# jonassibbesen/rpvg

Hardware: AMD Instinct MI355X
Metric: read-pairs quantified/sec (higher is better)
Workload: dtype f64

## Files before the change

### rpvg_amd/csrc/em_plan.hpp

```cpp
#ifndef RPVG_EM_PLAN_HPP
#define RPVG_EM_PLAN_HPP

#include <algorithm>
#include <cstddef>
#include <cstdint>

#ifndef RPVG_PLAN_FN
#if defined(__HIPCC__)
#define RPVG_PLAN_FN __host__ __device__ inline
#else
#define RPVG_PLAN_FN inline
#endif
#endif

namespace rpvg_em {

constexpr int kEmBins = 12;
constexpr int kEmGridBin = 11;
constexpr int kEmWideBin = 10;
constexpr int kEmWorkBuckets = 32;
constexpr uint32_t kEmMidGridMax = 8;
constexpr uint32_t kEmMidGridLog2 = 16;
constexpr uint32_t kEmMidBuckets = kEmWorkBuckets - kEmMidGridLog2;
constexpr int kEmStreamedBin = 3;
// ... 5 lines not shown

RPVG_PLAN_FN size_t emLdsBytes(uint32_t cols, uint32_t rows, uint32_t entries, int block, bool resident) {
    size_t bytes = sizeof(double) * ((1 + static_cast<size_t>(block) / 64) * cols + block / 64 + 2);
    if (resident) bytes += static_cast<size_t>(rows) * 16 + static_cast<size_t>(entries) * 8 + (static_cast<size_t>(rows) + 1 + entries) * 4 + 8;
    return (bytes + 15) & ~static_cast<size_t>(15);
}

RPVG_PLAN_FN size_t emGridLdsBytes(const uint32_t cols) { return sizeof(double) * 5 * static_cast<size_t>(cols); }

RPVG_PLAN_FN size_t emRegisterLdsBytes(const int rpl, const int cols) { return (64 * static_cast<size_t>(rpl) * cols + 2) * sizeof(double); }

struct EmBinRule {
    uint32_t use_register_kernel;
    uint64_t streamed_small_work;
    uint64_t grid_min_work;
};

RPVG_PLAN_FN int emBinOf(const EmBinRule rule, const uint32_t C, const uint32_t rows, const uint32_t entries) {
    const uint64_t work = static_cast<uint64_t>(entries) + rows;
    if (rule.grid_min_work != 0 && work >= rule.grid_min_work && emGridLdsBytes(C) <= kEmLdsLimit) return kEmGridBin;
    if (rule.use_register_kernel && C <= 16 && rows <= 256) return rows <= 64 ? 4 : rows <= 128 ? 5 : 6;
    if (rule.use_register_kernel && C <= kRegColsMax && rows <= 128) return rows <= 64 ? 8 : 9;
    if (emLdsBytes(C, rows, entries, 64, true) <= 8 * 1024) return 0;
    if (emLdsBytes(C, rows, entries, 256, true) <= 40 * 1024) return 1;
    if (emLdsBytes(C, rows, entries, 1024, true) <= 152 * 1024) return 7;
    if (emLdsBytes(C, 0, 0, 256, false) > kEmLdsLimit) return kEmWideBin;
    if (emLdsBytes(C, 0, 0, 1024, false) > kEmLdsLimit) return 2;
    return work <= rule.streamed_small_work ? 2 : 3;
}

RPVG_PLAN_FN uint32_t emWorkBucket(const uint32_t rows, const uint32_t entries) {
    uint64_t work = static_cast<uint64_t>(entries) + rows + 1;
    uint32_t lg = 0;
    while (work > 1 && lg < static_cast<uint32_t>(kEmWorkBuckets - 1)) {
        work >>= 1;
        ++lg;
    }
    return static_cast<uint32_t>(kEmWorkBuckets - 1) - lg;
}

RPVG_PLAN_FN bool emIsMidSize(const uint32_t bin, const uint32_t bucket) { return bin == static_cast<uint32_t>(kEmStreamedBin) && bucket < kEmMidBuckets; }
RPVG_PLAN_FN bool emMidGridAllowed(const uint64_t grid_min_work) { return grid_min_work > (1ull << kEmMidGridLog2); }
RPVG_PLAN_FN bool emMidGridMoves(const bool allowed, const uint32_t mid) { return allowed && mid > 0 && mid <= kEmMidGridMax; }
RPVG_PLAN_FN int emRouteOf(const int bin, const uint32_t bucket, const bool moved) {
    return moved && emIsMidSize(static_cast<uint32_t>(bin), bucket) ? kEmGridBin : bin;
}

RPVG_PLAN_FN bool emIsRegisterBin(const int bin) { return bin == 4 || bin == 5 || bin == 6 || bin == 8 || bin == 9; }
RPVG_PLAN_FN int emStatsSlot(const int bin, const bool one_register_launch) {
    return emIsRegisterBin(bin) && one_register_launch ? static_cast<int>(kRegisterKernelIndex) : bin;
}

constexpr int kEmMaxFusedDense = 4;
constexpr uint32_t kEmDenseMaxCols = 2048;
RPVG_PLAN_FN bool emDenseRule(const uint32_t columns, const uint32_t rows, const uint32_t entries) {
    if (columns > kEmDenseMaxCols || columns < 2) return false;
    const uint64_t ld = (static_cast<uint64_t>(columns) + 1) & ~1ull;
    return 8ull * rows * ld <= 12ull * entries + 20ull * rows;
}

constexpr uint32_t kLdsMapPaths = 16384;
constexpr uint32_t kFillSegmentRows = 1024;
constexpr uint64_t kFillLongRowEntries = 32;
constexpr size_t kFillLongRowLds = kFillSegmentRows * (3 * sizeof(uint32_t) + sizeof(double));
constexpr size_t kFillDenseLds = kFillSegmentRows * 2 * sizeof(uint32_t);
constexpr uint64_t kFillLongRowMinWork = 1ull << 18;
RPVG_PLAN_FN size_t emFillDenseLdsBytes(const uint32_t lds_map_paths, const uint64_t widest_ld) {
    return lds_map_paths * sizeof(int32_t) + kFillDenseLds + 4 * static_cast<size_t>(widest_ld) * sizeof(double);
}

struct EmSolveKnobs {
    EmBinRule rule = {1u, 0, 1ull << 18};
    bool no_collapse = false;
    bool no_fused_dense = false;
    bool register_copies = true;
    bool one_register_launch = true;
    bool fill_thread_rows = false;
    double grid_scale = 1.0;
    bool few_streams = false;
    bool launch_early = false;
    bool wait_sort_only = false;
    bool join_on_stream = false;
    bool collapse_debug = false;
    bool has_bound_bytes = false;
    uint64_t bound_bytes = 0;
};

RPVG_PLAN_FN bool emStorageByBound(const uint64_t rows_bound, const uint64_t entries_bound, const uint64_t budget) {
    return rows_bound * 20 + entries_bound * 12 <= budget;
}
template <typename Count>
inline void emStorageBases(const Count * rows, const Count * entries, const uint32_t P, uint64_t * row_base, uint64_t * ent_base, uint64_t * rows_total,
                           uint64_t * entries_total) {
    uint64_t r = 0, e = 0;
    for (uint32_t p = 0; p < P; ++p) {
        row_base[p] = r;
        ent_base[p] = e;
        r += rows[p];
        e += entries[p];
    }
    *rows_total = r;
    *entries_total = e;
}

constexpr size_t kGibbsOneWorkgroupLdsLimit = 160 * 1024;
RPVG_PLAN_FN size_t gibbsOneWorkgroupLds(const uint32_t columns) {
    return (sizeof(double) * (2 * static_cast<size_t>(columns) + 256 / 64 + 2) + 15) & ~static_cast<size_t>(15);
}
RPVG_PLAN_FN bool gibbsTakesGrid(const uint32_t columns, const uint32_t rows, const uint32_t entries, const uint64_t grid_min_work) {
    const bool too_wide = gibbsOneWorkgroupLds(columns) > kGibbsOneWorkgroupLdsLimit;
    const bool too_large = grid_min_work != 0 && static_cast<uint64_t>(rows) + entries >= grid_min_work;
    return too_wide || too_large;
}
RPVG_PLAN_FN bool gibbsGridPossible(const uint32_t max_cols, const uint64_t max_cluster_work, const uint64_t grid_min_work) {
    return gibbsOneWorkgroupLds(max_cols) > kGibbsOneWorkgroupLdsLimit || (grid_min_work != 0 && max_cluster_work >= grid_min_work);
}

struct EmSolveShape {
    uint32_t P = 0, items_bound = 0, max_cols = 0, max_cluster_paths = 0;
    uint64_t max_cluster_work = 0, rows_capacity = 0;
    unsigned long long wide_capacity = 0;
    uint32_t cus = 0;
    int side_streams = 6;
    int hardware_queues = 4;
    bool collapse_wanted = false;
};
constexpr int kEmSideStreams = 6;
constexpr uint32_t kEmCollapseMaxProblems = (1u << 20) - 2;
constexpr uint64_t kEmCollapseMaxRows = 0x7fffffffull;

struct EmFillPlan {
    uint32_t fill_grid = 0;
    uint32_t dense_grid = 0;
    uint32_t lds_map_paths = 0;
    bool long_row_scratch = false;
    size_t fill_lds = 0;
};
inline EmFillPlan planEmFill(const EmSolveShape & s, const EmSolveKnobs & knobs) {
    EmFillPlan f;
    f.fill_grid = std::min<uint32_t>(s.items_bound, s.cus * 8);
    f.dense_grid = std::min<uint32_t>(s.items_bound, s.cus * 4);
    f.lds_map_paths = (std::min<uint32_t>(s.max_cluster_paths, kLdsMapPaths) + 3) & ~3u;
    f.long_row_scratch = !knobs.fill_thread_rows && s.max_cluster_work >= kFillLongRowMinWork;
    f.fill_lds = f.lds_map_paths * sizeof(int32_t) + (f.long_row_scratch ? kFillLongRowLds : 0);
    return f;
}

enum class EmVariant : uint8_t {
    kSparse64Resident, kSparse256Resident, kSparse1024Resident, kSparse256Streamed, kSparse1024Streamed, kSparseWide,
    kRegisterBins,
    kRegister1x16, kRegister2x16, kRegister4x16, kRegister1x32, kRegister2x32
};
constexpr int kEmMainStream = -1;
struct EmLaunch {
    uint32_t bin;
    EmVariant variant;
    uint32_t grid;
    size_t lds;
    int stream;
};
inline bool operator==(const EmLaunch & a, const EmLaunch & b) {
    return a.bin == b.bin && a.variant == b.variant && a.grid == b.grid && a.lds == b.lds && a.stream == b.stream;
}
constexpr int kEmMaxLaunches = 11;

struct EmSolvePlan {
// ... 70 lines not shown
```

### rpvg_amd/csrc/em_sparse.hip

```cpp

#include "common.hpp"

#include "em_block.hpp"

#include <algorithm>
#include <memory>
#include <numeric>

using namespace rpvg_hip_detail;

namespace {

constexpr double kMinEmAbundance = 1e-8;
constexpr uint32_t kMinEmConvIts = 10;
static_assert(kEmBins == RPVG_HIP_EM_KERNELS, "a statistics slot per size bin (em_plan.hpp)");

struct EmQueues {
    uint32_t histogram[kEmBins * kEmWorkBuckets];
    uint32_t bucket_cursor[kEmBins * kEmWorkBuckets];
    uint32_t bin_start[kEmBins];
    uint32_t bin_count[kEmBins];
    uint32_t bin_cursor[kEmBins];
    uint32_t pad;
    unsigned long long wide_cursor;
    unsigned long long wide_overflow;
};


struct FillArgs {
    uint32_t num_problems;
    const uint32_t * num_problems_dev;
    uint32_t num_items;
    const uint32_t * num_items_dev;
    const uint64_t * seg_first;
    const uint32_t * item_problem;
    const uint32_t * prob_cluster;
    const uint32_t * col_path;
    const uint64_t * cluster_row_off;
    const uint64_t * cluster_path_off;
    const uint64_t * row_ent_off;
    const uint32_t * ent_path;
    const double * ent_prob;
    const double * row_count;
    const double * row_noise;
    EmProblemsView problems;
    uint32_t * seg_rows;
    uint32_t * seg_entries;
    double * seg_zero_mass;
    double * seg_total_mass;
    uint32_t * kept_entries;
    uint32_t * prob_bucket;
    EmQueues * queues;
    EmBinRule rule;
    uint32_t lds_map_paths;
    uint32_t long_row_scratch;
    uint32_t num_fused;
    EmFusedDense fused[kEmMaxFusedDense];
};

__device__ inline bool fillLongRows(const FillArgs & args, const uint32_t k) {
    const uint64_t c0 = args.cluster_row_off[k], c1 = args.cluster_row_off[k + 1];
    return args.long_row_scratch && args.row_ent_off[c1] - args.row_ent_off[c0] >= kFillLongRowEntries * (c1 - c0);
}

template <bool WRITE>
__global__ __launch_bounds__(256) void fillSegmentsKernel(const FillArgs args) {
    constexpr int BLOCK = 256;
    extern __shared__ __attribute__((aligned(16))) int32_t lds_map[];
    __shared__ uint32_t scratch[2 * (BLOCK / 64)];
    __shared__ double dscratch[BLOCK / 64];
    const uint32_t num_items = args.num_items_dev ? *args.num_items_dev : args.num_items;
    uint32_t mapped_problem = UINT32_MAX;
    for (uint32_t item = blockIdx.x; item < num_items; item += gridDim.x) {
        const uint32_t p = args.item_problem[item];
        if (WRITE) {
            bool fused = false;
            for (uint32_t f = 0; f < args.num_fused; ++f) fused = fused || args.fused[f].problem == p;
            if (fused) continue;
        }
        const uint32_t segment = static_cast<uint32_t>(item - args.seg_first[p]);
        const uint32_t k = args.prob_cluster[p];
        const uint32_t n_paths = static_cast<uint32_t>(args.cluster_path_off[k + 1] - args.cluster_path_off[k]);
        const uint32_t * cols = args.col_path + args.problems.col_off[p];
        const uint32_t n_cols = args.problems.paths(p);
        const bool use_map = n_paths <= args.lds_map_paths;
        const bool identity = n_cols == n_paths;
// ... 402 lines not shown
        if (c1 < kCells) start[c1] = excl + h0;
        if (threadIdx.x == 255) start[kCells] = before + incl;
    }
    __syncthreads();
    if (blockIdx.x == 0 && threadIdx.x < kEmBins) {
        queues->bin_start[threadIdx.x] = start[threadIdx.x * kEmWorkBuckets];
        queues->bin_count[threadIdx.x] = start[(threadIdx.x + 1) * kEmWorkBuckets] - start[threadIdx.x * kEmWorkBuckets];
    }
    const uint32_t p = blockIdx.x * blockDim.x + threadIdx.x;
    if (p >= P) return;
    uint32_t cell = prob_bucket[p];
    if (cell / kEmWorkBuckets == kEmStreamedBin && cell % kEmWorkBuckets < moved) cell = kEmGridBin * kEmWorkBuckets + cell % kEmWorkBuckets;
    order[start[cell] + atomicAdd(&queues->bucket_cursor[cell], 1u)] = p;
    if (cell / kEmWorkBuckets == 10) {
        const unsigned long long need = 2ull * (static_cast<unsigned long long>(col_off[p + 1] - col_off[p]) + 1);
        const unsigned long long at = atomicAdd(&queues->wide_cursor, need);
        wide_off[p] = at;
        if (at + need > wide_capacity) atomicAdd(&queues->wide_overflow, 1ull);
    }
}

struct GridDescribeArgs {
    const EmQueues * queues;
    const uint32_t * order;
    EmProblemsView problems;
    const uint32_t * kept_entries;
    EmGridProblem * out;
    uint32_t capacity;
};

__global__ __launch_bounds__(256) void emGridDescribeKernel(const GridDescribeArgs args) {
    const uint32_t i = blockIdx.x * blockDim.x + threadIdx.x;
    if (i >= args.queues->bin_count[kEmGridBin] || i >= args.capacity) return;
    const uint32_t p = args.order[args.queues->bin_start[kEmGridBin] + i];
    EmGridProblem d;
    d.problem = p;
    const EmProblemsView & v = args.problems;
    d.columns = v.paths(p) + 1;
    d.rows = v.kept_rows[p];
    d.entries = args.kept_entries[p];
    d.merged = (v.problem_merged != nullptr && v.problem_merged[p] != 0) ? 1u : 0u;
    d.pad = 0;
    d.row_base = v.row_base[p];
    d.ent_base = v.ent_base[p];
    d.col_begin = v.col_off[p];
    d.total_mass = v.total_mass[p];
    d.zero_mass = v.zero_mass[p];
    args.out[i] = d;
}


struct EmLaunchArgs {
    const uint32_t * order;
    EmQueues * queues;
    uint32_t bin;
    EmProblemsView problems;
    uint32_t max_em_its;
    uint32_t register_copies;
    double max_rel_em_conv;
    double * wide_vectors;
    const unsigned long long * wide_off;
    unsigned long long wide_capacity;
    double * abundances;
    double * noise_count;
    uint32_t * iterations;
};

template <int BLOCK>
__device__ __forceinline__ uint32_t nextProblem(const EmLaunchArgs & args, uint32_t * slot) {
    uint32_t i;
    if (BLOCK == 64) {
        i = (threadIdx.x == 0) ? atomicAdd(&args.queues->bin_cursor[args.bin], 1u) : 0u;
        i = static_cast<uint32_t>(__builtin_amdgcn_readfirstlane(static_cast<int>(i)));
    } else {
        __syncthreads();
        if (threadIdx.x == 0) *slot = atomicAdd(&args.queues->bin_cursor[args.bin], 1u);
        __syncthreads();
        i = *slot;
    }
    if (i >= args.queues->bin_count[args.bin]) return UINT32_MAX;
    return args.order[args.queues->bin_start[args.bin] + i];
}

template <int BLOCK, bool RESIDENT, bool WIDE>
__device__ __forceinline__ void emSparseProblem(const EmLaunchArgs & args, const uint32_t p, unsigned char * smem_raw) {
    const uint32_t C = args.problems.paths(p) + 1;
    if (WIDE && args.wide_off[p] + 2ull * C > args.wide_capacity) return;
    constexpr uint32_t kCopies = WIDE ? 1 : BLOCK / 64;
    double * a = WIDE ? args.wide_vectors + args.wide_off[p] : reinterpret_cast<double *>(smem_raw);
    double * t = a + C;
    double * red = WIDE ? reinterpret_cast<double *>(smem_raw) : t + static_cast<size_t>(kCopies) * C;
    double * tw = t + static_cast<size_t>(kCopies == 1 ? 0 : threadIdx.x >> 6) * C;

    const EmProblemRows csr = args.problems.mergedRows(p);
    const uint32_t n_rows = csr.rows;
    const uint32_t * off = csr.off;
    const double * cnt = csr.count;
    const double * nzv = csr.noise;
    const uint32_t * col = csr.col;
    const double * val = csr.val;
    if (RESIDENT) {
        const uint32_t n_ent = off[n_rows];
        double * l_cnt = red + (BLOCK / 64 + 2);
        double * l_nz = l_cnt + n_rows;
        double * l_val = l_nz + n_rows;
        uint32_t * l_off = reinterpret_cast<uint32_t *>(l_val + n_ent);
        uint32_t * l_col = l_off + (n_rows + 1);
        for (uint32_t r = threadIdx.x; r < n_rows; r += BLOCK) {
            l_cnt[r] = cnt[r];
            l_nz[r] = nzv[r];
        }
        for (uint32_t r = threadIdx.x; r <= n_rows; r += BLOCK) l_off[r] = off[r];
        for (uint32_t e = threadIdx.x; e < n_ent; e += BLOCK) {
            l_val[e] = val[e];
            l_col[e] = col[e];
        }
        off = l_off;
        cnt = l_cnt;
        nzv = l_nz;
        col = l_col;
        val = l_val;
    }
    const double T = args.problems.total_mass[p];
    const double Z = args.problems.zero_mass[p];
    const double eps = args.max_rel_em_conv;
    const uint32_t noise_col = C - 1;

    const double a0 = static_cast<double>(1.0f / static_cast<float>(C));
    for (uint32_t j = threadIdx.x; j < C; j += BLOCK) a[j] = a0;

    for (uint32_t j = threadIdx.x; j < kCopies * C; j += BLOCK) t[j] = 0;
    __syncthreads();

    const double inv_T = 1.0 / T;
    uint32_t iters = 0, conv = 0;
    for (uint32_t it = 0; it < args.max_em_its; ++it) {
        const double a_noise = a[noise_col];
        double tn = 0;
        for (uint32_t r = threadIdx.x; r < n_rows; r += BLOCK) {
            const uint32_t e0 = off[r], e1 = off[r + 1];
            const double nz = nzv[r];
            double s = nz * a_noise;
            for (uint32_t e = e0; e < e1; ++e) s += val[e] * a[col[e]];
            double y = __builtin_amdgcn_rcp(s);
            y = fma(fma(-s, y, 1.0), y, y);
            y = fma(fma(-s, y, 1.0), y, y);
            const double quot = cnt[r] * y;
            const double w = cnt[r] == 0.0 ? 0.0 : fma(fma(-s, quot, cnt[r]), y, quot);
            for (uint32_t e = e0; e < e1; ++e) atomicAdd(&tw[col[e]], w * val[e]);
            tn += w * nz;
        }
        tn = waveSumF64(tn);
        if ((threadIdx.x & 63) == 0 && tn != 0.0) atomicAdd(&tw[noise_col], tn);
        __syncthreads();
        int viol = 0;
        for (uint32_t j = threadIdx.x; j < C; j += BLOCK) {
            const double aj = a[j];
            double tj = t[j];
            t[j] = 0;
#pragma unroll
            for (uint32_t w = 1; w < kCopies; ++w) {
                tj += t[w * C + j];
                t[w * C + j] = 0;
            }
            const double an = (j == noise_col) ? (aj * tj + Z) * inv_T : (aj * tj) * inv_T;
            if (an >= kMinEmAbundance && fabs(an - aj) > eps * an) viol = 1;
            a[j] = an;
        }
        int any_viol;
        if (BLOCK == 64) {
            any_viol = __any(viol);
            __syncthreads();
        } else {
            any_viol = __syncthreads_or(viol);
        }
        ++iters;
        if (!any_viol) {
            if (++conv == kMinEmConvIts) break;
        } else {
            conv = 0;
        }
    }

    double low = 0;
    double * out = args.abundances + args.problems.col_off[p];
    for (uint32_t j = threadIdx.x; j < noise_col; j += BLOCK) {
        const double aj = a[j];
        if (aj < kMinEmAbundance) {
            low += aj * T;
            out[j] = 0;
        } else {
            out[j] = aj * T;
        }
    }
    low = blockReduceSum<double, BLOCK>(low, red);
    if (threadIdx.x == 0) {
        args.noise_count[p] = low + a[noise_col] * T;
        args.iterations[p] = iters;
    }
}

template <int BLOCK, bool RESIDENT, bool WIDE = false>
__global__ __launch_bounds__(BLOCK) void emSparseKernel(const EmLaunchArgs args) {
    extern __shared__ __attribute__((aligned(16))) unsigned char smem_raw[];
    __shared__ uint32_t next_slot;
    if (blockIdx.x >= args.queues->bin_count[args.bin]) return;
    for (uint32_t p = nextProblem<BLOCK>(args, &next_slot); p != UINT32_MAX; p = nextProblem<BLOCK>(args, &next_slot)) {
        emSparseProblem<BLOCK, RESIDENT, WIDE>(args, p, smem_raw);
        if (BLOCK == 64) __syncthreads();
    }
}

template <int BLOCK, bool RESIDENT, bool WIDE = false>
hipError_t launchEm(const EmLaunchArgs & args, uint32_t grid, size_t lds, hipStream_t stream) {
    if (grid == 0) return hipSuccess;
    if (lds > kLdsOptIn) {
        hipError_t e = hipFuncSetAttribute(reinterpret_cast<const void *>(&emSparseKernel<BLOCK, RESIDENT, WIDE>),
                                           hipFuncAttributeMaxDynamicSharedMemorySize, static_cast<int>(lds));
        if (e != hipSuccess) return e;
    }
    emSparseKernel<BLOCK, RESIDENT, WIDE><<<dim3(grid), dim3(BLOCK), lds, stream>>>(args);
    return hipGetLastError();
}


template <int D>
__device__ __forceinline__ double quadSwapF64(const double v) {
    constexpr int perm = (D == 1) ? 0xB1 : 0x4E;
    const int lo = __builtin_amdgcn_mov_dpp(__double2loint(v), perm, 0xF, 0xF, true);
    const int hi = __builtin_amdgcn_mov_dpp(__double2hiint(v), perm, 0xF, 0xF, true);
    return __hiloint2double(hi, lo);
}

__device__ __forceinline__ void swapHalvesF64(double & x, double & y) {
    const auto lo = __builtin_amdgcn_permlane32_swap(static_cast<unsigned>(__double2loint(x)), static_cast<unsigned>(__double2loint(y)), false, false);
    const auto hi = __builtin_amdgcn_permlane32_swap(static_cast<unsigned>(__double2hiint(x)), static_cast<unsigned>(__double2hiint(y)), false, false);
    x = __hiloint2double(static_cast<int>(hi[0]), static_cast<int>(lo[0]));
    y = __hiloint2double(static_cast<int>(hi[1]), static_cast<int>(lo[1]));
}

__device__ __forceinline__ void swapRowsF64(double & x, double & y) {
    const auto lo = __builtin_amdgcn_permlane16_swap(static_cast<unsigned>(__double2loint(x)), static_cast<unsigned>(__double2loint(y)), false, false);
    const auto hi = __builtin_amdgcn_permlane16_swap(static_cast<unsigned>(__double2hiint(x)), static_cast<unsigned>(__double2hiint(y)), false, false);
    x = __hiloint2double(static_cast<int>(hi[0]), static_cast<int>(lo[0]));
    y = __hiloint2double(static_cast<int>(hi[1]), static_cast<int>(lo[1]));
}

template <int CTRL>
__device__ __forceinline__ double halveF64(const double x, const double y, const bool upper) {
    const double send = upper ? x : y, keep = upper ? y : x;
    const int lo = __builtin_amdgcn_mov_dpp(__double2loint(send), CTRL, 0xF, 0xF, true);
    const int hi = __builtin_amdgcn_mov_dpp(__double2hiint(send), CTRL, 0xF, 0xF, true);
    return keep + __hiloint2double(hi, lo);
}

template <int COLS, int SKIP = 0>
__device__ __forceinline__ double columnSumsOverWave(double (&v)[COLS], const uint32_t lane) {
    if (SKIP < 1) {
#pragma unroll
        for (int c = 0; c < COLS / 2; ++c) {
            swapHalvesF64(v[c], v[c + COLS / 2]);
            v[c] += v[c + COLS / 2];
        }
    }
    if (SKIP < 2) {
#pragma unroll
        for (int c = 0; c < COLS / 4; ++c) {
            swapRowsF64(v[c], v[c + COLS / 4]);
            v[c] += v[c + COLS / 4];
        }
    }
    const bool bit3 = (lane & 8) != 0, bit2 = (lane & 4) != 0;
#pragma unroll
    for (int c = 0; c < COLS / 8; ++c) v[c] = halveF64<0x128>(v[c], v[c + COLS / 8], bit3);
#pragma unroll
    for (int c = 0; c < COLS / 16; ++c) v[c] = halveF64<0x141>(v[c], v[c + COLS / 16], bit2);
    double t;
    if (COLS == 32) {
        t = halveF64<0x4E>(v[0], v[1], (lane & 2) != 0);
    } else {
        t = v[0];
        t += quadSwapF64<2>(t);
    }
    t += quadSwapF64<1>(t);
    return t;
}

template <int RPL, int COLS, int COPIES = 1>
__device__ __forceinline__ void emRegisterProblem(const EmLaunchArgs & args, const uint32_t p, double * reg_lds) {
    static_assert(COPIES == 1 || (RPL == 1 && COLS == 16), "copies: one row per lane, 16 columns");
    constexpr uint32_t kCols = COLS;
    constexpr int kSkip = COPIES == 4 ? 2 : (COPIES == 2 ? 1 : 0);
    constexpr int kShare = COLS / COPIES;
    constexpr int kLanesPerColumn = 64 / COLS;
    const uint32_t np = args.problems.paths(p);
    const uint32_t lane = threadIdx.x;
    const EmProblemRows csr = args.problems.mergedRows(p);
    const uint32_t n_rows = csr.rows;
    const uint32_t * off = csr.off;
    const double * cnt = csr.count;
    const double * nzv = csr.noise;
    const uint32_t * col = csr.col;
    const double * val = csr.val;

    constexpr uint32_t kTile = 64 * RPL * kCols;
// ... 98 lines not shown
}

template <int RPL, int COLS>
__device__ __forceinline__ void emRegisterBin(const EmLaunchArgs & args, const uint32_t block, double * reg_lds) {
    if (block >= args.queues->bin_count[args.bin]) return;
    for (uint32_t p = nextProblem<64>(args, nullptr); p != UINT32_MAX; p = nextProblem<64>(args, nullptr)) {
        if (RPL == 1 && COLS == 16 && args.register_copies) {
            const uint32_t n_rows = args.problems.kept_rows[p];
            if (n_rows <= 16) emRegisterProblem<1, 16, 4>(args, p, reg_lds);
            else if (n_rows <= 32) emRegisterProblem<1, 16, 2>(args, p, reg_lds);
            else emRegisterProblem<1, 16, 1>(args, p, reg_lds);
        } else {
            emRegisterProblem<RPL, COLS>(args, p, reg_lds);
        }
        __syncthreads();
    }
}

template <int RPL, int COLS>
__global__ __launch_bounds__(64) void emRegisterBinKernel(const EmLaunchArgs args) {
    extern __shared__ __attribute__((aligned(16))) double reg_lds[];
    emRegisterBin<RPL, COLS>(args, blockIdx.x, reg_lds);
}


__global__ __launch_bounds__(64) void emRegisterKernel(const EmLaunchArgs launch_args, const uint32_t variants) {
    extern __shared__ __attribute__((aligned(16))) double reg_lds[];
    EmLaunchArgs args = launch_args;
    const uint32_t variant = blockIdx.x % variants, block = blockIdx.x / variants;
    args.bin = kRegisterBins[variant];
    switch (variant) {
        case 0: emRegisterBin<4, 16>(args, block, reg_lds); break;
        case 1: emRegisterBin<1, 16>(args, block, reg_lds); break;
        case 2: emRegisterBin<2, 16>(args, block, reg_lds); break;
        case 3: emRegisterBin<1, 32>(args, block, reg_lds); break;
        default: emRegisterBin<2, 32>(args, block, reg_lds); break;
    }
}

template <int RPL, int COLS>
hipError_t launchEmRegister(const EmLaunchArgs & args, uint32_t grid, size_t lds, hipStream_t stream) {
    if (grid == 0) return hipSuccess;
    emRegisterBinKernel<RPL, COLS><<<dim3(grid), dim3(64), lds, stream>>>(args);
    return hipGetLastError();
}

hipError_t launchEmRegisterBins(const EmLaunchArgs & args, const uint32_t grid_per_bin, const bool with_32_columns, const size_t lds, hipStream_t stream) {
    if (grid_per_bin == 0) return hipSuccess;
    const uint32_t variants = with_32_columns ? 5u : 3u;
    emRegisterKernel<<<dim3(grid_per_bin * variants), dim3(64), lds, stream>>>(args, variants);
    return hipGetLastError();
}

}

namespace rpvg_hip_detail {

size_t emQueuesBytes() { return sizeof(EmQueues); }
uint32_t emFillSegmentRows() { return kFillSegmentRows; }

EmSolveKnobs emSolveKnobs() {
    static const EmSolveKnobs once = []() {
        EmSolveKnobs k;
        k.rule.use_register_kernel = RPVG_EXPERIMENT_ENV("RPVG_HIP_NO_REGISTER_EM") == nullptr ? 1u : 0u;
        k.rule.streamed_small_work = RPVG_EXPERIMENT_ENV("RPVG_HIP_EM_STREAM_SMALL") ? std::strtoull(RPVG_EXPERIMENT_ENV("RPVG_HIP_EM_STREAM_SMALL"), nullptr, 10) : 0;
        k.no_collapse = RPVG_EXPERIMENT_ENV("RPVG_HIP_NO_EM_COLLAPSE") != nullptr;
        const char * launches = std::getenv("RPVG_HIP_EM_REGISTER_LAUNCHES");
        k.one_register_launch = !(launches && std::atoi(launches) == 5);
        k.fill_thread_rows = RPVG_EXPERIMENT_ENV("RPVG_HIP_FILL_THREAD_ROWS") != nullptr;
        k.grid_scale = RPVG_EXPERIMENT_ENV("RPVG_HIP_EM_GRID_SCALE") ? std::atof(RPVG_EXPERIMENT_ENV("RPVG_HIP_EM_GRID_SCALE")) : 1.0;
        k.few_streams = RPVG_EXPERIMENT_ENV("RPVG_HIP_EM_FEW_STREAMS") != nullptr;
        k.launch_early = RPVG_EXPERIMENT_ENV("RPVG_HIP_EM_LAUNCH_EARLY") != nullptr;
        k.wait_sort_only = RPVG_EXPERIMENT_ENV("RPVG_HIP_EM_WAIT_SORT_ONLY") != nullptr;
        k.join_on_stream = RPVG_EXPERIMENT_ENV("RPVG_HIP_EM_JOIN_ON_STREAM") != nullptr;
        k.collapse_debug = RPVG_EXPERIMENT_ENV("RPVG_HIP_EM_COLLAPSE_DEBUG") != nullptr;
        return k;
    }();
    EmSolveKnobs k = once;
    k.rule.grid_min_work = emGridMinWork();
    k.no_collapse = k.no_collapse || RPVG_EXPERIMENT_ENV("RPVG_HIP_NO_COLLAPSE") != nullptr;
    k.no_fused_dense = std::getenv("RPVG_HIP_NO_FUSED_DENSE") != nullptr;
    const char * copies = std::getenv("RPVG_HIP_EM_COPIES");
    k.register_copies = copies ? std::atoi(copies) != 0 : true;
    const char * budget = std::getenv("RPVG_HIP_EM_BOUND_BYTES");
    k.has_bound_bytes = budget != nullptr;
    k.bound_bytes = budget ? static_cast<uint64_t>(std::atof(budget)) : 0;
    return k;
}

EmSolveShape emSolveShape(const rpvg_hip_ctx * ctx, const EmProblemList & list, const bool collapse_wanted) {
    EmSolveShape s;
    s.P = list.P_bound;
    s.items_bound = list.items_bound;
    s.max_cols = list.max_cols;
    s.max_cluster_paths = list.max_cluster_paths;
    s.max_cluster_work = list.max_cluster_work;
    s.rows_capacity = list.rows_capacity;
    s.wide_capacity = list.wide_capacity;
    s.cus = static_cast<uint32_t>(ctx->props.multiProcessorCount);
    s.side_streams = ctx->aux_count;
    s.hardware_queues = hardwareQueues();
    s.collapse_wanted = collapse_wanted;
    return s;
}

}

namespace {

static_assert(kEmSideStreams == rpvg_hip_ctx::kAuxStreams && kEmCollapseMaxProblems + 2 == kCollapseMaxMatrices, "em_plan.hpp restates these");

struct EmCountBuffers {
    DeviceBuffer<uint32_t> * seg_rows, * seg_entries;
    DeviceBuffer<double> * seg_zero, * seg_total;
};

int queueEmCount(rpvg_hip_ctx * ctx, const rpvg_hip_batch * batch, const EmProblemList & list, const EmOutputs & out, const EmProblemsView & view,
                 const EmCountBuffers & buffers, const EmBinRule rule, EmQueues * queues, uint32_t * prob_bucket, const EmFillPlan & plan, FillArgs & fa) {
    hipStream_t st = ctx->stream;
    RPVG_HIP_CHECK(buffers.seg_rows->alloc(list.items_bound));
    RPVG_HIP_CHECK(buffers.seg_entries->alloc(list.items_bound));
    RPVG_HIP_CHECK(buffers.seg_zero->alloc(list.items_bound));
    RPVG_HIP_CHECK(buffers.seg_total->alloc(list.items_bound));
    fa = FillArgs{};
    fa.num_problems = list.P_bound;
    fa.num_problems_dev = list.d_num_problems;
    fa.num_items = list.items_bound;
    fa.num_items_dev = list.d_num_items;
    fa.seg_first = list.d_seg_first;
    fa.item_problem = list.d_item_problem;
    fa.prob_cluster = list.d_cluster;
    fa.col_path = list.d_col_path;
    fa.cluster_row_off = batch->cluster_row_off.ptr;
    fa.cluster_path_off = batch->cluster_path_off.ptr;
    fa.row_ent_off = batch->row_ent_off.ptr;
    fa.ent_path = batch->ent_path.ptr;
    fa.ent_prob = batch->ent_prob.ptr;
    fa.row_count = batch->row_count.ptr;
    fa.row_noise = batch->row_noise.ptr;
    fa.problems = view;
    fa.seg_rows = buffers.seg_rows->ptr;
    fa.seg_entries = buffers.seg_entries->ptr;
    fa.seg_zero_mass = buffers.seg_zero->ptr;
    fa.seg_total_mass = buffers.seg_total->ptr;
    fa.kept_entries = out.d_kept_entries;
    fa.prob_bucket = prob_bucket;
    fa.queues = queues;
    fa.rule = rule;
    fa.lds_map_paths = plan.lds_map_paths;
    fa.long_row_scratch = plan.long_row_scratch ? 1u : 0u;
    fa.num_fused = 0;
    RPVG_HIP_CHECK(launchFillSegments<false>(fa, plan, st));
    fillOffsetsKernel<<<dim3((list.P_bound + 255) / 256), dim3(256), 0, st>>>(fa);
    return RPVG_HIP_OK;
}

int lookForFusedDense(rpvg_hip_ctx * ctx, const uint32_t P, EmSolveWork & work, FillArgs & fa) {
    hipStream_t st = ctx->stream;
    DeviceBuffer<DenseCandidates> d_candidates;
    DenseCandidates * h_candidates = nullptr;
    RPVG_HIP_CHECK(d_candidates.alloc(1));
    if (pinnedAlloc(reinterpret_cast<void **>(&h_candidates), sizeof(DenseCandidates)) != hipSuccess) {
        setError("rpvg_hip_em_solve: out of page-locked host memory");
        return RPVG_HIP_ERR_ALLOC;
    }
    struct PinnedGuard {
// ... 32 lines not shown

namespace rpvg_hip_detail {

int queueEmFill(rpvg_hip_ctx * ctx, const rpvg_hip_batch * batch, const EmProblemList & list, const EmOutputs & out, EmSolveWork & work,
                const EmSolveKnobs & knobs, const EmFillPlan & plan, const bool fused_look, int & build_span) {
    hipStream_t st = ctx->stream;
    const uint32_t P = list.P_bound;
    RPVG_HIP_CHECK(work.d_prow_off.alloc(list.rows_capacity + P));
    RPVG_HIP_CHECK(work.d_prow_count.alloc(list.rows_capacity));
    RPVG_HIP_CHECK(work.d_prow_noise.alloc(list.rows_capacity));
    RPVG_HIP_CHECK(work.d_pent_col.alloc(list.entries_capacity));
    RPVG_HIP_CHECK(work.d_pent_val.alloc(list.entries_capacity));
    RPVG_HIP_CHECK(work.d_zero.alloc(P));
    RPVG_HIP_CHECK(work.d_bucket.alloc(P));
    RPVG_HIP_CHECK(work.d_order.alloc(P));
    if (!work.zeroed_queues) RPVG_HIP_CHECK(work.d_queues.alloc(sizeof(EmQueues)));
    if (list.wide_capacity > 0) {
        RPVG_HIP_CHECK(work.d_wide_vectors.alloc(list.wide_capacity));
        RPVG_HIP_CHECK(work.d_wide_off.alloc(P));
    }
    build_span = ctx->spanBegin(FAM_BUILD);
    if (!work.zeroed_queues) RPVG_HIP_CHECK(zeroAsync(work.d_queues.ptr, sizeof(EmQueues), st));
    FillArgs fa;
    const EmCountBuffers buffers{&work.d_seg_rows, &work.d_seg_entries, &work.d_seg_zero, &work.d_seg_total};
    const int rc = queueEmCount(ctx, batch, list, out, work.view(list, out), buffers, knobs.rule, queuesOf(work), work.d_bucket.ptr, plan, fa);
    if (rc != RPVG_HIP_OK) return rc;
    if (fused_look) {
        const int look = lookForFusedDense(ctx, P, work, fa);
        if (look != RPVG_HIP_OK) return look;
    }
    RPVG_HIP_CHECK(launchFillSegments<true>(fa, plan, st));
    if (fa.num_fused > 0) {
        uint64_t widest = 0;
        for (uint32_t f = 0; f < fa.num_fused; ++f) widest = std::max(widest, fa.fused[f].ld);
        const size_t lds = emFillDenseLdsBytes(fa.lds_map_paths, widest);
        if (lds > kLdsOptIn) RPVG_HIP_CHECK(hipFuncSetAttribute(reinterpret_cast<const void *>(&fillDenseRowsKernel), hipFuncAttributeMaxDynamicSharedMemorySize, static_cast<int>(lds)));
        fillDenseRowsKernel<<<dim3(plan.dense_grid, fa.num_fused), dim3(256), lds, st>>>(fa);
        RPVG_HIP_CHECK(hipGetLastError());
        ctx->stats.build_launches += 1;
    }
    RPVG_HIP_CHECK(hipGetLastError());
    ctx->stats.build_launches += 3;
    return RPVG_HIP_OK;
}

}

namespace {

int queueEmCollapse(rpvg_hip_ctx * ctx, const EmProblemList & list, const EmSolvePlan & plan, const EmSolveKnobs & knobs, const double precision,
                    EmSolveWork & work, EmProblemsView & view, std::unique_ptr<HostScope> & stage_scope) {
    auto cw = std::make_shared<CsrCollapseWork>();
    work.collapse = cw;
    RPVG_HIP_CHECK(hipEventCreateWithFlags(&work.collapsed, hipEventDisableTiming));
    RPVG_HIP_CHECK(hipStreamWaitEvent(ctx->collapse_stream, work.filled, 0));
    CsrCollapseInput in;
    in.num_problems_bound = list.P_bound;
    in.num_problems_dev = list.d_num_problems;
    in.rows_capacity = list.rows_capacity;
    in.problems = view;
    in.num_items_bound = list.items_bound;
    in.num_items_dev = list.d_num_items;
    in.seg_first = list.d_seg_first;
    in.item_problem = list.d_item_problem;
    in.segment_rows = kFillSegmentRows;
    in.max_rows_bound = plan.collapse_max_rows;
    const int collapse_span = ctx->spanBegin(FAM_COLLAPSE, ctx->collapse_stream);
    RPVG_HIP_CHECK(hipEventCreateWithFlags(&work.collapse_sorted, hipEventDisableTiming));
    stage_scope.reset(new HostScope("em_solve: the problems' collapse queued"));
    RPVG_HIP_CHECK(queueCsrCollapse(ctx, in, precision, *cw, ctx->collapse_stream, work.collapse_sorted));
    stage_scope.reset(new HostScope("em_solve: EM launches, grid problems, join"));
    ctx->spanEnd(collapse_span);
    RPVG_HIP_CHECK(hipEventRecord(work.collapsed, ctx->collapse_stream));
    view.merged_count = cw->merged_count.ptr;
    view.problem_merged = cw->problem_merged.ptr;
    RPVG_HIP_CHECK(hipStreamWaitEvent(ctx->stream, work.collapsed, 0));
    if (!knobs.launch_early && work.collapse_sorted) {
        HostScope wait_scope("em_solve: wait for the collapse");
        RPVG_HIP_CHECK(waitEvent(knobs.wait_sort_only ? work.collapse_sorted : work.collapsed));
    }
    return RPVG_HIP_OK;
}

int queueEmLaunches(rpvg_hip_ctx * ctx, const EmSolvePlan & plan, EmLaunchArgs & args) {
    RPVG_HIP_CHECK(ctx->forkAux());
    for (int i = 0; i < plan.num_launches; ++i) {
        const EmLaunch & l = plan.launches[i];
        hipStream_t on = l.stream == kEmMainStream ? ctx->stream : ctx->aux[l.stream];
        args.bin = l.bin;
        const int bin_span = ctx->spanBegin(FAM_EM_KERNEL, on, static_cast<int>(l.bin));
        hipError_t e = hipSuccess;
        switch (l.variant) {
            case EmVariant::kSparse64Resident: e = launchEm<64, true>(args, l.grid, l.lds, on); break;
            case EmVariant::kSparse256Resident: e = launchEm<256, true>(args, l.grid, l.lds, on); break;
            case EmVariant::kSparse1024Resident: e = launchEm<1024, true>(args, l.grid, l.lds, on); break;
            case EmVariant::kSparse256Streamed: e = launchEm<256, false>(args, l.grid, l.lds, on); break;
            case EmVariant::kSparse1024Streamed: e = launchEm<1024, false>(args, l.grid, l.lds, on); break;
            case EmVariant::kSparseWide: e = launchEm<1024, false, true>(args, l.grid, l.lds, on); break;
            case EmVariant::kRegisterBins: e = launchEmRegisterBins(args, l.grid, plan.with_32_columns, l.lds, on); break;
            case EmVariant::kRegister1x16: e = launchEmRegister<1, 16>(args, l.grid, l.lds, on); break;
            case EmVariant::kRegister2x16: e = launchEmRegister<2, 16>(args, l.grid, l.lds, on); break;
            case EmVariant::kRegister4x16: e = launchEmRegister<4, 16>(args, l.grid, l.lds, on); break;
            case EmVariant::kRegister1x32: e = launchEmRegister<1, 32>(args, l.grid, l.lds, on); break;
            case EmVariant::kRegister2x32: e = launchEmRegister<2, 32>(args, l.grid, l.lds, on); break;
        }
        RPVG_HIP_CHECK(e);
        ctx->spanEnd(bin_span);
    }
    return RPVG_HIP_OK;
}

struct EmGridLook {
    DeviceBuffer<EmGridProblem> d_problems;
    hipEvent_t described = nullptr;
    uint32_t * h_count = nullptr;
    ~EmGridLook() {
        if (described) (void) hipEventDestroy(described);
        if (h_count) pinnedFree(h_count);
    }
};
int queueEmGridLook(rpvg_hip_ctx * ctx, const uint32_t P, const EmProblemsView & view, const EmOutputs & out, const EmSolveWork & work, EmGridLook & look) {
    hipStream_t st = ctx->stream;
    EmQueues * queues = queuesOf(work);
    RPVG_HIP_CHECK(look.d_problems.alloc(P));
    if (pinnedAlloc(reinterpret_cast<void **>(&look.h_count), 64) != hipSuccess) {
        setError("rpvg_hip_em_solve: out of page-locked host memory");
        return RPVG_HIP_ERR_ALLOC;
    }
    GridDescribeArgs da;
    da.queues = queues;
    da.order = work.d_order.ptr;
    da.problems = view;
    da.kept_entries = out.d_kept_entries;
    da.out = look.d_problems.ptr;
    da.capacity = P;
    emGridDescribeKernel<<<dim3((P + 255) / 256), dim3(256), 0, st>>>(da);
    RPVG_HIP_CHECK(hipGetLastError());
    RPVG_HIP_CHECK(hipMemcpyAsync(look.h_count, &queues->bin_count[kEmGridBin], sizeof(uint32_t), hipMemcpyDeviceToHost, st));
    RPVG_HIP_CHECK(hipEventCreateWithFlags(&look.described, hipEventDisableTiming));
    RPVG_HIP_CHECK(hipEventRecord(look.described, st));
    return RPVG_HIP_OK;
}

int queueEmGridAndJoin(rpvg_hip_ctx * ctx, const uint32_t P, const EmProblemsView & view, const EmOutputs & out, const EmSolveWork & work,
                       const EmSolveKnobs & knobs, EmGridLook * look, const uint32_t max_em_its, const double max_rel_em_conv) {
    hipStream_t st = ctx->stream;
    if (look) {
        RPVG_HIP_CHECK(waitEvent(look->described));
        const uint32_t n_grid = std::min<uint32_t>(*look->h_count, P);
        if (n_grid > 0) {
            std::vector<EmGridProblem> grid_problems(n_grid);
            RPVG_HIP_CHECK(hipMemcpyAsync(grid_problems.data(), look->d_problems.ptr, sizeof(EmGridProblem) * n_grid, hipMemcpyDeviceToHost, st));
            RPVG_HIP_CHECK(waitStream(st));
            EmGridStorage storage;
            storage.problems = view;
            storage.abundances = out.d_abundances;
            storage.noise_count = out.d_noise_count;
            storage.iterations = out.d_iterations;
            storage.fused = work.fused;
            storage.num_fused = work.num_fused;
            const int rc = runEmGridProblems(ctx, st, grid_problems.data(), n_grid, storage, max_em_its, max_rel_em_conv);
            if (rc != RPVG_HIP_OK) return rc;
        }
    }
    RPVG_HIP_CHECK(knobs.join_on_stream ? ctx->joinAux() : ctx->joinAuxOnHost());
    return RPVG_HIP_OK;
}

int dumpEmCollapse(rpvg_hip_ctx * ctx, const EmProblemList & list, const EmSolveWork & work) {
    const CsrCollapseWork * cw = static_cast<const CsrCollapseWork *>(work.collapse.get());
    const uint32_t P = list.P_bound;
    uint32_t info[6] = {0}, merged = 0, problems = P, counts[3] = {0};
    RPVG_HIP_CHECK(waitStream(ctx->stream));
    RPVG_HIP_CHECK(hipMemcpy(info, cw->info.ptr, sizeof(info), hipMemcpyDeviceToHost));
    RPVG_HIP_CHECK(hipMemcpy(&merged, cw->problem_merged.ptr + P, sizeof(merged), hipMemcpyDeviceToHost));
    if (list.d_num_problems) RPVG_HIP_CHECK(hipMemcpy(&problems, list.d_num_problems, sizeof(problems), hipMemcpyDeviceToHost));
    {
        const uint64_t mark_words = (list.rows_capacity + 31) / 32;
        RPVG_HIP_CHECK(hipMemcpy(counts, cw->info.ptr + 6 + 2 + 2 * static_cast<uint64_t>(P) + 1 + mark_words, sizeof(counts), hipMemcpyDeviceToHost));
    }
    std::fprintf(stderr, "[em collapse] marked rows %u forward pairs %u (equal up to rounding %u, apart %u) around pairs %u\n", counts[0], counts[1], info[4], info[5], counts[2]);
    std::fprintf(stderr, "[em collapse] problems %u (bound %u) row slots %llu: replayed %u whole %u active rows %u rows replaced %u problems merged %u\n",
                 problems, P, static_cast<unsigned long long>(list.rows_capacity), info[0], info[2], info[3], info[1], merged);
    return RPVG_HIP_OK;
}

}

namespace rpvg_hip_detail {

int queueEmSolve(rpvg_hip_ctx * ctx, const rpvg_hip_batch * batch, const EmProblemList & list, const uint32_t max_em_its,
                 const double max_rel_em_conv, const EmOutputs & out, EmSolveWork & work, const double collapse_precision) {
    hipStream_t st = ctx->stream;
    const uint32_t P = list.P_bound;
    const EmSolveKnobs knobs = emSolveKnobs();
    const EmSolvePlan plan = planEmSolve(emSolveShape(ctx, list, collapse_precision > 0), knobs);
    std::unique_ptr<HostScope> stage_scope(new HostScope("em_solve: allocations + fill queued"));
    int span = -1;
    int rc = queueEmFill(ctx, batch, list, out, work, knobs, plan.fill, plan.fused_look, span);
    if (rc != RPVG_HIP_OK) return rc;
    RPVG_REQUIRE(!plan.collapse_too_large,
                 "EM solve with a row collapse: %llu row slots in %u problems exceed what one solve can collapse (2^31 - 1 rows, 2^20 - 2 problems): split the problem list",
                 static_cast<unsigned long long>(list.rows_capacity), P);
    if (plan.collapse) {
        RPVG_HIP_CHECK(hipEventCreateWithFlags(&work.filled, hipEventDisableTiming));
        RPVG_HIP_CHECK(hipEventRecord(work.filled, st));
    }
    emOrderKernel<<<dim3((P + 255) / 256), dim3(256), 0, st>>>(P, list.d_num_problems, work.d_bucket.ptr, list.d_col_off, queuesOf(work), work.d_order.ptr,
                                                              work.d_wide_off.ptr, list.wide_capacity, plan.mid_grid_allowed ? 1u : 0u);
    RPVG_HIP_CHECK(hipGetLastError());
    ctx->spanEnd(span);
    ctx->stats.build_launches += 1;

    EmProblemsView view = work.view(list, out);
    if (plan.collapse) {
        rc = queueEmCollapse(ctx, list, plan, knobs, collapse_precision, work, view, stage_scope);
        if (rc != RPVG_HIP_OK) return rc;
    }

    EmLaunchArgs args;
    args.order = work.d_order.ptr;
    args.queues = queuesOf(work);
    args.bin = 0;
    args.problems = view;
    args.max_em_its = max_em_its;
    args.register_copies = knobs.register_copies ? 1u : 0u;
    args.max_rel_em_conv = max_rel_em_conv;
    args.wide_vectors = work.d_wide_vectors.ptr;
    args.wide_off = work.d_wide_off.ptr;
    args.wide_capacity = list.wide_capacity;
    args.abundances = out.d_abundances;
    args.noise_count = out.d_noise_count;
    args.iterations = out.d_iterations;

    EmGridLook look;
    if (plan.grid_possible) {
        rc = queueEmGridLook(ctx, P, view, out, work, look);
        if (rc != RPVG_HIP_OK) return rc;
    }
    span = ctx->spanBegin(FAM_EM_SPARSE);
    rc = queueEmLaunches(ctx, plan, args);
    if (rc != RPVG_HIP_OK) return rc;
    rc = queueEmGridAndJoin(ctx, P, view, out, work, knobs, plan.grid_possible ? &look : nullptr, max_em_its, max_rel_em_conv);
    if (rc != RPVG_HIP_OK) return rc;
    ctx->spanEnd(span);
    if (plan.collapse && knobs.collapse_debug) return dumpEmCollapse(ctx, list, work);
    return RPVG_HIP_OK;
}

void accountEmSolve(rpvg_hip_ctx * ctx, const uint32_t P, const uint64_t * col_off, const uint32_t * kept_rows, const uint32_t * kept_entries,
                    const uint32_t * iterations) {
    const EmSolveKnobs knobs = emSolveKnobs();
    const EmBinRule rule = knobs.rule;
    double bin_bytes[kEmBins] = {};
    uint64_t bin_its[kEmBins] = {}, bin_problems[kEmBins] = {};
    uint32_t bin_slowest[kEmBins] = {};
    uint32_t mid_problems = 0;
    for (uint32_t p = 0; p < P; ++p) {
        const uint32_t C = static_cast<uint32_t>(col_off[p + 1] - col_off[p]) + 1;
        if (emIsMidSize(static_cast<uint32_t>(emBinOf(rule, C, kept_rows[p], kept_entries[p])), emWorkBucket(kept_rows[p], kept_entries[p]))) ++mid_problems;
    }
    const bool mid_moved = emMidGridMoves(emMidGridAllowed(rule.grid_min_work), mid_problems);
    for (uint32_t p = 0; p < P; ++p) {
        const uint32_t C = static_cast<uint32_t>(col_off[p + 1] - col_off[p]) + 1;
        const int b = emRouteOf(emBinOf(rule, C, kept_rows[p], kept_entries[p]), emWorkBucket(kept_rows[p], kept_entries[p]), mid_moved);
        if (b == kEmGridBin && emGridDenseRoute(C, kept_rows[p], kept_entries[p])) {
            bin_problems[b] += 1;
            continue;
        }
        bin_bytes[b] += static_cast<double>(iterations[p]) * (12.0 * kept_entries[p] + 20.0 * kept_rows[p] + 16.0 * C);
        bin_its[b] += iterations[p];
        bin_problems[b] += 1;
        bin_slowest[b] = std::max(bin_slowest[b], iterations[p]);
    }
    double slot_bytes[kEmBins] = {};
    uint64_t slot_its[kEmBins] = {}, slot_problems[kEmBins] = {};
    uint32_t slot_slowest[kEmBins] = {};
    for (int b = 0; b < kEmBins; ++b) {
        const int slot = emStatsSlot(b, knobs.one_register_launch);
        slot_bytes[slot] += bin_bytes[b];
        slot_its[slot] += bin_its[b];
        slot_problems[slot] += bin_problems[b];
        slot_slowest[slot] = std::max(slot_slowest[slot], bin_slowest[b]);
    }
    for (int b = 0; b < kEmBins; ++b) {
        if (!slot_problems[b]) continue;
        rpvg_hip_em_kernel_stats & ks = ctx->stats.em_kernel[b];
        ks.launches += 1;
        ks.problems += slot_problems[b];
        ks.iterations += slot_its[b];
        ks.max_iterations += slot_slowest[b];
        ks.alg_bytes += slot_bytes[b];
        ctx->stats.em_sparse_launches += 1;
        ctx->stats.em_sparse_alg_bytes += slot_bytes[b];
        ctx->stats.em_iterations_total += slot_its[b];
    }
}

namespace {
uint64_t deviceMemoryBudget() {
    static const uint64_t budget = []() {
        size_t free_bytes = 0, total_bytes = 0;
        if (hipMemGetInfo(&free_bytes, &total_bytes) != hipSuccess) {
            (void) hipGetLastError();
            return static_cast<uint64_t>(4ull << 30);
        }
        return static_cast<uint64_t>(free_bytes) * 2 / 5;
    }();
    return budget;
}
}

int prepareHostProblems(rpvg_hip_ctx * ctx, const rpvg_hip_batch * batch, const rpvg_hip_em_problems * problems,
                        HostProblemSet & ps, const EmOutputs & out, const char * who) {
    const uint32_t P = problems->num_problems;
    std::unique_ptr<HostScope> scope(new HostScope("problems: validate"));
    std::vector<uint64_t> row_base(P), ent_base(P), cluster_rows(P), cluster_entries(P);
    EmProblemList & list = ps.list;
    for (uint32_t p = 0; p < P; ++p) {
        const uint32_t k = problems->cluster[p];
        RPVG_REQUIRE(k < batch->num_clusters, "%s: problem %u refers to cluster %u of %u", who, p, k, batch->num_clusters);
        const uint64_t n_paths = batch->h_cluster_path_off[k + 1] - batch->h_cluster_path_off[k];
        const uint64_t c0 = problems->col_off[p], c1 = problems->col_off[p + 1];
        RPVG_REQUIRE(c1 > c0, "%s: problem %u has no columns", who, p);
// ... 130 lines not shown
```

Baseline: 2.347 billion.

## Interleave multiple rows per thread in sparse EM with batched loads and gathers

```diff
diff --git a/rpvg_amd/csrc/em_plan.hpp b/rpvg_amd/csrc/em_plan.hpp
--- a/rpvg_amd/csrc/em_plan.hpp
+++ b/rpvg_amd/csrc/em_plan.hpp
@@ -111,6 +111,7 @@
     bool wait_sort_only = false;
     bool join_on_stream = false;
     bool collapse_debug = false;
+    bool plain_rows = false;
     bool has_bound_bytes = false;
     uint64_t bound_bytes = 0;
 };
diff --git a/rpvg_amd/csrc/em_rows.hpp b/rpvg_amd/csrc/em_rows.hpp
--- /dev/null
+++ b/rpvg_amd/csrc/em_rows.hpp
@@ -0,0 +1,85 @@
+#ifndef RPVG_EM_ROWS_HPP
+#define RPVG_EM_ROWS_HPP
+
+#include <cstdint>
+
+#ifndef RPVG_PLAN_FN
+#if defined(__HIPCC__)
+#define RPVG_PLAN_FN __host__ __device__ inline
+#else
+#define RPVG_PLAN_FN inline
+#endif
+#endif
+
+#if defined(__clang__)
+#define RPVG_ROWS_UNROLL _Pragma("unroll")
+#else
+#define RPVG_ROWS_UNROLL
+#endif
+
+namespace rpvg_em {
+
+constexpr int kEmRowsWeightStages = 4;
+
+template <int BLOCK, bool RESIDENT>
+struct EmRowsShape {
+    static constexpr int U = BLOCK >= 1024 ? 2 : BLOCK <= 64 ? 3 : RESIDENT ? 2 : 4;
+    static constexpr int H = 4;
+};
+
+template <int U, int H, class Lane>
+RPVG_PLAN_FN void emRowsWalk(const uint32_t tid, const uint32_t block, const uint32_t n_rows, const uint32_t n_ent, Lane & lane) {
+    for (uint32_t first = tid; first < n_rows; first += static_cast<uint32_t>(U) * block) {
+        bool live[U];
+        uint32_t n[U];
+        RPVG_ROWS_UNROLL
+        for (int u = 0; u < U; ++u) {
+            const uint32_t r = first + static_cast<uint32_t>(u) * block;
+            live[u] = r < n_rows;
+            const uint32_t entries = lane.head(u, live[u] ? r : first);
+            n[u] = live[u] ? entries : 0u;
+        }
+        RPVG_ROWS_UNROLL
+        for (int u = 0; u < U; ++u) lane.start(u);
+        if (n_ent != 0) {
+            RPVG_ROWS_UNROLL
+            for (int u = 0; u < U; ++u) {
+                RPVG_ROWS_UNROLL
+                for (int j = 0; j < H; ++j) lane.load(u, j, static_cast<uint32_t>(j) < n[u]);
+            }
+            RPVG_ROWS_UNROLL
+            for (int u = 0; u < U; ++u) {
+                RPVG_ROWS_UNROLL
+                for (int j = 0; j < H; ++j) lane.gather(u, j);
+            }
+            RPVG_ROWS_UNROLL
+            for (int j = 0; j < H; ++j) {
+                RPVG_ROWS_UNROLL
+                for (int u = 0; u < U; ++u) lane.sumHeld(u, j, static_cast<uint32_t>(j) < n[u]);
+            }
+            RPVG_ROWS_UNROLL
+            for (int u = 0; u < U; ++u) {
+                for (uint32_t j = H; j < n[u]; ++j) lane.sumTail(u, j);
+            }
+        }
+        RPVG_ROWS_UNROLL
+        for (int stage = 0; stage < kEmRowsWeightStages; ++stage) {
+            RPVG_ROWS_UNROLL
+            for (int u = 0; u < U; ++u) lane.weight(u, stage);
+        }
+        RPVG_ROWS_UNROLL
+        for (int u = 0; u < U; ++u) {
+            if (!live[u]) continue;
+            RPVG_ROWS_UNROLL
+            for (int j = 0; j < H; ++j) {
+                if (static_cast<uint32_t>(j) < n[u]) lane.addHeld(u, j);
+            }
+            for (uint32_t j = H; j < n[u]; ++j) lane.addTail(u, j);
+            lane.addNoise(u);
+        }
+    }
+}
+
+}
+
+#endif
diff --git a/rpvg_amd/csrc/em_sparse.hip b/rpvg_amd/csrc/em_sparse.hip
--- a/rpvg_amd/csrc/em_sparse.hip
+++ b/rpvg_amd/csrc/em_sparse.hip
@@ -2,6 +2,7 @@
 #include "common.hpp"
 
 #include "em_block.hpp"
+#include "em_rows.hpp"
 
 #include <algorithm>
 #include <memory>
@@ -570,7 +571,54 @@
     return args.order[args.queues->bin_start[args.bin] + i];
 }
 
-template <int BLOCK, bool RESIDENT, bool WIDE>
+template <int U, int H>
+struct EmRowsLane {
+    const uint32_t * off;
+    const double * cnt;
+    const double * nzv;
+    const uint32_t * col;
+    const double * val;
+    const double * a;
+    double * tw;
+    double a_noise;
+    double tn;
+    uint32_t e0[U];
+    double nz[U], c[U], s[U], y[U], w[U];
+    double v[U][H], av[U][H];
+    uint32_t cl[U][H];
+
+    __device__ __forceinline__ uint32_t head(const int u, const uint32_t r) {
+        e0[u] = off[r];
+        const uint32_t e1 = off[r + 1];
+        nz[u] = nzv[r];
+        c[u] = cnt[r];
+        return e1 - e0[u];
+    }
+    __device__ __forceinline__ void load(const int u, const int j, const bool held) {
+        const uint32_t e = held ? e0[u] + j : 0u;
+        v[u][j] = val[e];
+        cl[u][j] = col[e];
+    }
+    __device__ __forceinline__ void gather(const int u, const int j) { av[u][j] = a[cl[u][j]]; }
+    __device__ __forceinline__ void start(const int u) { s[u] = __dmul_rn(nz[u], a_noise); }
+    __device__ __forceinline__ void sumHeld(const int u, const int j, const bool held) { s[u] = held ? fma(v[u][j], av[u][j], s[u]) : s[u]; }
+    __device__ __forceinline__ void sumTail(const int u, const uint32_t j) { s[u] = fma(val[e0[u] + j], a[col[e0[u] + j]], s[u]); }
+    __device__ __forceinline__ void weight(const int u, const int stage) {
+        if (stage == 0) {
+            y[u] = __builtin_amdgcn_rcp(s[u]);
+        } else if (stage < 3) {
+            y[u] = fma(fma(-s[u], y[u], 1.0), y[u], y[u]);
+        } else {
+            const double quot = __dmul_rn(c[u], y[u]);
+            w[u] = c[u] == 0.0 ? 0.0 : fma(fma(-s[u], quot, c[u]), y[u], quot);
+        }
+    }
+    __device__ __forceinline__ void addHeld(const int u, const int j) { atomicAdd(&tw[cl[u][j]], __dmul_rn(w[u], v[u][j])); }
+    __device__ __forceinline__ void addTail(const int u, const uint32_t j) { atomicAdd(&tw[col[e0[u] + j]], __dmul_rn(w[u], val[e0[u] + j])); }
+    __device__ __forceinline__ void addNoise(const int u) { tn = fma(w[u], nz[u], tn); }
+};
+
+template <int BLOCK, bool RESIDENT, bool WIDE, bool PLAIN>
 __device__ __forceinline__ void emSparseProblem(const EmLaunchArgs & args, const uint32_t p, unsigned char * smem_raw) {
     const uint32_t C = args.problems.paths(p) + 1;
     if (WIDE && args.wide_off[p] + 2ull * C > args.wide_capacity) return;
@@ -625,7 +673,22 @@
     for (uint32_t it = 0; it < args.max_em_its; ++it) {
         const double a_noise = a[noise_col];
         double tn = 0;
-        for (uint32_t r = threadIdx.x; r < n_rows; r += BLOCK) {
+        if (!PLAIN) {
+            using Shape = rpvg_em::EmRowsShape<BLOCK, RESIDENT>;
+            EmRowsLane<Shape::U, Shape::H> lane;
+            lane.off = off;
+            lane.cnt = cnt;
+            lane.nzv = nzv;
+            lane.col = col;
+            lane.val = val;
+            lane.a = a;
+            lane.tw = tw;
+            lane.a_noise = a_noise;
+            lane.tn = 0;
+            rpvg_em::emRowsWalk<Shape::U, Shape::H>(threadIdx.x, BLOCK, n_rows, off[n_rows], lane);
+            tn = lane.tn;
+        }
+        for (uint32_t r = threadIdx.x; PLAIN && r < n_rows; r += BLOCK) {
             const uint32_t e0 = off[r], e1 = off[r + 1];
             const double nz = nzv[r];
             double s = nz * a_noise;
@@ -688,27 +751,32 @@
     }
 }
 
-template <int BLOCK, bool RESIDENT, bool WIDE = false>
+template <int BLOCK, bool RESIDENT, bool WIDE = false, bool PLAIN = WIDE>
 __global__ __launch_bounds__(BLOCK) void emSparseKernel(const EmLaunchArgs args) {
     extern __shared__ __attribute__((aligned(16))) unsigned char smem_raw[];
     __shared__ uint32_t next_slot;
     if (blockIdx.x >= args.queues->bin_count[args.bin]) return;
     for (uint32_t p = nextProblem<BLOCK>(args, &next_slot); p != UINT32_MAX; p = nextProblem<BLOCK>(args, &next_slot)) {
-        emSparseProblem<BLOCK, RESIDENT, WIDE>(args, p, smem_raw);
+        emSparseProblem<BLOCK, RESIDENT, WIDE, PLAIN>(args, p, smem_raw);
         if (BLOCK == 64) __syncthreads();
     }
 }
 
-template <int BLOCK, bool RESIDENT, bool WIDE = false>
+template <int BLOCK, bool RESIDENT, bool WIDE = false, bool PLAIN = WIDE>
 hipError_t launchEm(const EmLaunchArgs & args, uint32_t grid, size_t lds, hipStream_t stream) {
     if (grid == 0) return hipSuccess;
     if (lds > kLdsOptIn) {
-        hipError_t e = hipFuncSetAttribute(reinterpret_cast<const void *>(&emSparseKernel<BLOCK, RESIDENT, WIDE>),
+        hipError_t e = hipFuncSetAttribute(reinterpret_cast<const void *>(&emSparseKernel<BLOCK, RESIDENT, WIDE, PLAIN>),
                                            hipFuncAttributeMaxDynamicSharedMemorySize, static_cast<int>(lds));
         if (e != hipSuccess) return e;
     }
-    emSparseKernel<BLOCK, RESIDENT, WIDE><<<dim3(grid), dim3(BLOCK), lds, stream>>>(args);
+    emSparseKernel<BLOCK, RESIDENT, WIDE, PLAIN><<<dim3(grid), dim3(BLOCK), lds, stream>>>(args);
     return hipGetLastError();
+}
+
+template <int BLOCK, bool RESIDENT>
+hipError_t launchEmRows(const EmLaunchArgs & args, uint32_t grid, size_t lds, hipStream_t stream, const bool plain_rows) {
+    return plain_rows ? launchEm<BLOCK, RESIDENT, false, true>(args, grid, lds, stream) : launchEm<BLOCK, RESIDENT, false, false>(args, grid, lds, stream);
 }
 
 
@@ -973,6 +1041,8 @@
     k.no_fused_dense = std::getenv("RPVG_HIP_NO_FUSED_DENSE") != nullptr;
     const char * copies = std::getenv("RPVG_HIP_EM_COPIES");
     k.register_copies = copies ? std::atoi(copies) != 0 : true;
+    const char * plain_rows = std::getenv("RPVG_HIP_EM_PLAIN_ROWS");
+    k.plain_rows = plain_rows && std::atoi(plain_rows) != 0;
     const char * budget = std::getenv("RPVG_HIP_EM_BOUND_BYTES");
     k.has_bound_bytes = budget != nullptr;
     k.bound_bytes = budget ? static_cast<uint64_t>(std::atof(budget)) : 0;
@@ -1171,7 +1241,7 @@
     return RPVG_HIP_OK;
 }
 
-int queueEmLaunches(rpvg_hip_ctx * ctx, const EmSolvePlan & plan, EmLaunchArgs & args) {
+int queueEmLaunches(rpvg_hip_ctx * ctx, const EmSolvePlan & plan, const EmSolveKnobs & knobs, EmLaunchArgs & args) {
     RPVG_HIP_CHECK(ctx->forkAux());
     for (int i = 0; i < plan.num_launches; ++i) {
         const EmLaunch & l = plan.launches[i];
@@ -1180,11 +1250,11 @@
         const int bin_span = ctx->spanBegin(FAM_EM_KERNEL, on, static_cast<int>(l.bin));
         hipError_t e = hipSuccess;
         switch (l.variant) {
-            case EmVariant::kSparse64Resident: e = launchEm<64, true>(args, l.grid, l.lds, on); break;
-            case EmVariant::kSparse256Resident: e = launchEm<256, true>(args, l.grid, l.lds, on); break;
-            case EmVariant::kSparse1024Resident: e = launchEm<1024, true>(args, l.grid, l.lds, on); break;
-            case EmVariant::kSparse256Streamed: e = launchEm<256, false>(args, l.grid, l.lds, on); break;
-            case EmVariant::kSparse1024Streamed: e = launchEm<1024, false>(args, l.grid, l.lds, on); break;
+            case EmVariant::kSparse64Resident: e = launchEmRows<64, true>(args, l.grid, l.lds, on, knobs.plain_rows); break;
+            case EmVariant::kSparse256Resident: e = launchEmRows<256, true>(args, l.grid, l.lds, on, knobs.plain_rows); break;
+            case EmVariant::kSparse1024Resident: e = launchEmRows<1024, true>(args, l.grid, l.lds, on, knobs.plain_rows); break;
+            case EmVariant::kSparse256Streamed: e = launchEmRows<256, false>(args, l.grid, l.lds, on, knobs.plain_rows); break;
+            case EmVariant::kSparse1024Streamed: e = launchEmRows<1024, false>(args, l.grid, l.lds, on, knobs.plain_rows); break;
             case EmVariant::kSparseWide: e = launchEm<1024, false, true>(args, l.grid, l.lds, on); break;
             case EmVariant::kRegisterBins: e = launchEmRegisterBins(args, l.grid, plan.with_32_columns, l.lds, on); break;
             case EmVariant::kRegister1x16: e = launchEmRegister<1, 16>(args, l.grid, l.lds, on); break;
@@ -1328,7 +1398,7 @@
         if (rc != RPVG_HIP_OK) return rc;
     }
     span = ctx->spanBegin(FAM_EM_SPARSE);
-    rc = queueEmLaunches(ctx, plan, args);
+    rc = queueEmLaunches(ctx, plan, knobs, args);
     if (rc != RPVG_HIP_OK) return rc;
     rc = queueEmGridAndJoin(ctx, P, view, out, work, knobs, plan.grid_possible ? &look : nullptr, max_em_its, max_rel_em_conv);
     if (rc != RPVG_HIP_OK) return rc;
```

Result: no change. 2.344 billion (-0.1%).
